# xswang/xflow

Measured on NVIDIA H100. Metric: training examples/sec, higher is better.
Workload: dtype f32

## Files before the change

xflow_b200/csrc/step_lazy.cu:

```cuda
#include <cuda_runtime.h>
#include <stdint.h>
#include <stdlib.h>

#include "kernels.h"
#include "table.cuh"

#define XF_NO_SLOT 0xFFFFFFFFu
#define XF_LAZY_CACHED 2

template <bool ADMIT, bool STAMP>
__device__ __forceinline__ bool xf_lazy_look(const XfTableView& t, uint64_t key, uint64_t& s, uint32_t& i, uint64_t& q0,
                                             uint64_t& q1, uint64_t& q2, uint64_t& q3, uint32_t& slot, bool& created,
                                             const XfAdmitView& adm, bool& rejected, const XfStampView& sv) {
  if (q0 == key) { slot = (uint32_t)s; return true; }
  if (q0 == XF_EMPTY_KEY) {
    if (ADMIT && !xf_admit(adm, key)) {
      rejected = adm.mode != XF_ADM_NEVER;
      return true;
    }
    const unsigned long long old =
        atomicCAS(reinterpret_cast<unsigned long long*>(xf_row(t, s)), (unsigned long long)XF_EMPTY_KEY, (unsigned long long)key);
    if (old == XF_EMPTY_KEY) {
      if (STAMP) sv.stamp[s] = sv.now;
      created = true;
      q0 = key; q1 = q2 = q3 = 0ull;
      slot = (uint32_t)s;
      return true;
    }
    if (old == key) {
      q0 = key;
      slot = (uint32_t)s;
      return true;
    }
  }
  if (++i == XF_MAX_PROBE) { *t.error = 1; return true; }
  s = xf_probe_slot(t, key, i);
  return false;
}

template <bool ADMIT, bool STAMP, bool WEIGHT>
__global__ void __launch_bounds__(256, 3)
xf_k_step_lr_lazy(XfTableView t, const uint32_t* __restrict__ row_ptr, const uint64_t* __restrict__ keys,
                  const uint8_t* __restrict__ labels, int B, int mode, uint32_t seq, uint64_t* rows_by_seq, int fix_shift,
                  float* __restrict__ loss_out, float* __restrict__ pctr_out, float* __restrict__ abs_loss_sum,
                  unsigned long long* __restrict__ unique_total, XfAdmitView adm, XfStampView sv, XfWeightView wv) {
  __shared__ float s_abs[8];
  __shared__ unsigned int s_open;
  if (WEIGHT) fix_shift = xf_fix_shift(*wv.W);
  __shared__ uint64_t s_q2[2 * XF_LAZY_CACHED][256], s_q3[2 * XF_LAZY_CACHED][256], s_q2n[2 * XF_LAZY_CACHED][256];
  if (threadIdx.x == 0) s_open = 0;
  if (blockIdx.x == 0 && threadIdx.x == 0 && mode == 0)
    rows_by_seq[seq] = (uint64_t)(uint32_t)B | ((uint64_t)fix_shift << 32);
  __syncthreads();
  float abs_acc = 0.f;
  unsigned int open_acc = 0;
  const int lane = threadIdx.x & 31;
  const int warps_per_block = blockDim.x >> 5;
  const int gwarp = blockIdx.x * warps_per_block + (threadIdx.x >> 5);
  const int nwarps = gridDim.x * warps_per_block;

  for (int row = gwarp; row < B; row += nwarps) {
    if (WEIGHT && __ldg(wv.e + row) == 0.f) {
      if (lane == 0 && loss_out) loss_out[row] = 0.f;
      continue;
    }
    const uint32_t beg = __ldg(row_ptr + row);
    const uint32_t end = __ldg(row_ptr + row + 1);
    const int chunks = (int)((end - beg + 63u) >> 6);
    float wsum = 0.f;
    uint32_t lead_s[2 * XF_LAZY_CACHED];
    uint32_t cnt_c[XF_LAZY_CACHED];
#pragma unroll
    for (int c = 0; c < XF_LAZY_CACHED; ++c) {
      lead_s[2 * c] = lead_s[2 * c + 1] = XF_NO_SLOT;
      cnt_c[c] = 0;
    }

    for (int ch = 0; ch < chunks; ++ch) {
      const uint32_t j0 = beg + (uint32_t)ch * 64u + (uint32_t)lane;
      const uint32_t j1 = j0 + 32u;
      const bool v0 = j0 < end, v1 = j1 < end;
      const uint64_t k0 = v0 ? __ldcs(keys + j0) : 0ull;
      const uint64_t k1 = v1 ? __ldcs(keys + j1) : 0ull;
      uint64_t p0 = xf_home_slot(t, k0), p1 = xf_home_slot(t, k1);
      uint64_t a0, a1, a2, a3, b0, b1, b2, b3;
      xf_ld32_pair(v0 ? xf_row(t, p0) : nullptr, a0, a1, a2, a3);
      xf_ld32_pair(v1 ? xf_row(t, p1) : nullptr, b0, b1, b2, b3);
      uint32_t s0 = XF_NO_SLOT, s1 = XF_NO_SLOT, i0 = 0, i1 = 0;
      bool u0 = v0, u1 = v1, r0 = false, r1 = false;
      for (;;) {
        bool c0 = false, c1 = false;
        if (u0) u0 = !xf_lazy_look<ADMIT, STAMP>(t, k0, p0, i0, a0, a1, a2, a3, s0, c0, adm, r0, sv);
        if (u1) u1 = !xf_lazy_look<ADMIT, STAMP>(t, k1, p1, i1, b0, b1, b2, b3, s1, c1, adm, r1, sv);
        const unsigned created = __popc(__ballot_sync(0xffffffffu, c0)) + __popc(__ballot_sync(0xffffffffu, c1));
        if (created && lane == 0) {
          atomicAdd(t.size, (unsigned long long)created);
          if (ADMIT) atomicAdd(adm.admitted, (unsigned long long)created);
        }
        if (!__any_sync(0xffffffffu, u0 || u1)) break;
        uint64_t x0, x1, x2, x3;
        xf_ld32_pair(u0 ? xf_row(t, p0) : nullptr, x0, x1, x2, x3);
        if (u0) { a0 = x0; a1 = x1; a2 = x2; a3 = x3; }
        xf_ld32_pair(u1 ? xf_row(t, p1) : nullptr, x0, x1, x2, x3);
        if (u1) { b0 = x0; b1 = x1; b2 = x2; b3 = x3; }
      }
      if (ADMIT) xf_admit_append(adm, r0, k0, r1, k1);
      uint64_t a2n = a2, b2n = b2;
      float w0 = 0.f, w1 = 0.f;
      if (s0 != XF_NO_SLOT) w0 = xf_lazy_fold(t, a1, a2, a3, mode == 1 ? 0xFFFFFFFFu : seq, a2n);
      if (s1 != XF_NO_SLOT) w1 = xf_lazy_fold(t, b1, b2, b3, mode == 1 ? 0xFFFFFFFFu : seq, b2n);
      wsum += w0;
      wsum += w1;
      if (mode == 1) continue;
      const unsigned grp0 = __match_any_sync(0xffffffffu, (s0 != XF_NO_SLOT) ? s0 : (0xFFFFFF00u | (uint32_t)lane));
      const unsigned grp1 = __match_any_sync(0xffffffffu, (s1 != XF_NO_SLOT) ? s1 : (0xFFFFFF00u | (uint32_t)lane));
      const bool L0 = s0 != XF_NO_SLOT && lane == __ffs(grp0) - 1, L1 = s1 != XF_NO_SLOT && lane == __ffs(grp1) - 1;
      if (ch >= XF_LAZY_CACHED) {
        if (L0 && xf_lazy_deposit(t, xf_row(t, s0), a2, a3, a2n, seq, 0ll)) {
          ++open_acc;
          if (STAMP) sv.stamp[s0] = sv.now;
        }
        if (L1 && xf_lazy_deposit(t, xf_row(t, s1), b2, b3, b2n, seq, 0ll)) {
          ++open_acc;
          if (STAMP) sv.stamp[s1] = sv.now;
        }
      }
#pragma unroll
      for (int c = 0; c < XF_LAZY_CACHED; ++c)
        if (ch == c) {
          lead_s[2 * c] = L0 ? s0 : XF_NO_SLOT;
          lead_s[2 * c + 1] = L1 ? s1 : XF_NO_SLOT;
          cnt_c[c] = (L0 ? (uint32_t)__popc(grp0) : 0u) | ((L1 ? (uint32_t)__popc(grp1) : 0u) << 8);
        }
      if (ch < XF_LAZY_CACHED) {
        if (L0) { s_q2[2 * ch][threadIdx.x] = a2; s_q3[2 * ch][threadIdx.x] = a3; s_q2n[2 * ch][threadIdx.x] = a2n; }
        if (L1) { s_q2[2 * ch + 1][threadIdx.x] = b2; s_q3[2 * ch + 1][threadIdx.x] = b3; s_q2n[2 * ch + 1][threadIdx.x] = b2n; }
      }
    }

    const float wx = xf_warp_sum(wsum);
    const float pctr = xf_sigmoid(wx);
    if (mode == 1) {
      if (lane == 0 && pctr_out) pctr_out[row] = pctr;
      continue;
    }
    float loss = __fsub_rn(pctr, (float)labels[row]);
    if (lane == 0 && loss_out) loss_out[row] = loss;
    if (WEIGHT) loss = __fmul_rn(__ldg(wv.e + row), loss);
    abs_acc += fabsf(loss);
    const long long lf = xf_fix_of(loss, fix_shift);
#pragma unroll
    for (int c = 0; c < XF_LAZY_CACHED; ++c) {
      const int x = threadIdx.x;
      if (lead_s[2 * c] != XF_NO_SLOT &&
          xf_lazy_deposit(t, xf_row(t, lead_s[2 * c]), s_q2[2 * c][x], s_q3[2 * c][x], s_q2n[2 * c][x], seq,
                          lf * (long long)(cnt_c[c] & 0xFFu))) {
        ++open_acc;
        if (STAMP) sv.stamp[lead_s[2 * c]] = sv.now;
      }
      if (lead_s[2 * c + 1] != XF_NO_SLOT &&
          xf_lazy_deposit(t, xf_row(t, lead_s[2 * c + 1]), s_q2[2 * c + 1][x], s_q3[2 * c + 1][x], s_q2n[2 * c + 1][x], seq,
                          lf * (long long)(cnt_c[c] >> 8))) {
        ++open_acc;
        if (STAMP) sv.stamp[lead_s[2 * c + 1]] = sv.now;
      }
    }
    for (int ch = XF_LAZY_CACHED; ch < chunks; ++ch) {
      const uint32_t j0 = beg + (uint32_t)ch * 64u + (uint32_t)lane;
      const uint32_t j1 = j0 + 32u;
      XfHead h;
      if (j0 < end) { const int64_t r = xf_probe<false>(t, __ldg(keys + j0), &h); if (r >= 0) xf_lazy_add(xf_row(t, (uint64_t)r), lf); }
      if (j1 < end) { const int64_t r = xf_probe<false>(t, __ldg(keys + j1), &h); if (r >= 0) xf_lazy_add(xf_row(t, (uint64_t)r), lf); }
    }
  }
  if (mode == 0) {
    if (lane == 0) s_abs[threadIdx.x >> 5] = abs_acc;
    if (open_acc) atomicAdd(&s_open, open_acc);
    __syncthreads();
    if (threadIdx.x == 0) {
      if (abs_loss_sum != nullptr) {
        float tot = 0.f;
        for (int w = 0; w < (int)(blockDim.x >> 5); ++w) tot += s_abs[w];
        atomicAdd(abs_loss_sum, tot);
      }
      if (unique_total != nullptr && s_open) atomicAdd(unique_total, (unsigned long long)s_open);
    }
  }
}

void xf_launch_step_lr_lazy(const XfTableView& t, const uint32_t* row_ptr, const uint64_t* keys,
                            const uint8_t* labels, int B, uint64_t nnz, int mode, uint32_t seq, uint64_t* rows_by_seq,
                            float* loss_out, float* pctr_out, float* abs_loss_sum, unsigned long long* unique_total,
                            const XfAdmitView* adm, const XfStampView& sv, const XfWeightView& wv, cudaStream_t st) {
  if (B <= 0) return;
  const int grid = xf_grid_for((uint64_t)B * 32, 256, 8);
  const int fs = xf_fix_shift(nnz);
  const XfAdmitView a = adm ? *adm : XfAdmitView{};
#define XF_LAZY_ARGS t, row_ptr, keys, labels, B, mode, seq, rows_by_seq, fs, loss_out, pctr_out, abs_loss_sum, unique_total, a, sv, wv
#define XF_LAZY_LAUNCH(A, S)                                                       \
  do {                                                                             \
    if (wv.e) xf_k_step_lr_lazy<A, S, true><<<grid, 256, 0, st>>>(XF_LAZY_ARGS);   \
    else xf_k_step_lr_lazy<A, S, false><<<grid, 256, 0, st>>>(XF_LAZY_ARGS);       \
  } while (0)
  const bool stamp = sv.stamp != nullptr;
  if (adm && stamp) XF_LAZY_LAUNCH(true, true);
  else if (adm) XF_LAZY_LAUNCH(true, false);
  else if (stamp) XF_LAZY_LAUNCH(false, true);
  else XF_LAZY_LAUNCH(false, false);
#undef XF_LAZY_LAUNCH
#undef XF_LAZY_ARGS
}
```

Baseline: 83.03 million.

## Prefetch second-chunk keys, split lazy deposits into issue/resolve, size grid by occupancy

Loads each row's label and its second chunk of keys before the first chunk's probe loop, so those loads overlap with hashing. Splits the cached-lead deposits into an issue phase for all groups followed by a resolve phase, so their memory operations can be in flight together. Relaxes launch bounds from 3 to 2 blocks per SM to allow more registers, and computes the grid from the measured occupancy instead of a fixed 8 blocks per SM. Holding the extra prefetched keys and in-flight values raises register pressure, and stale resolutions now set an error flag.

```diff
diff --git a/xflow_b200/csrc/step_lazy.cu b/xflow_b200/csrc/step_lazy.cu
--- a/xflow_b200/csrc/step_lazy.cu
+++ b/xflow_b200/csrc/step_lazy.cu
@@ -39,7 +39,7 @@
 }
 
 template <bool ADMIT, bool STAMP, bool WEIGHT>
-__global__ void __launch_bounds__(256, 3)
+__global__ void __launch_bounds__(256, 2)
 xf_k_step_lr_lazy(XfTableView t, const uint32_t* __restrict__ row_ptr, const uint64_t* __restrict__ keys,
                   const uint8_t* __restrict__ labels, int B, int mode, uint32_t seq, uint64_t* rows_by_seq, int fix_shift,
                   float* __restrict__ loss_out, float* __restrict__ pctr_out, float* __restrict__ abs_loss_sum,
@@ -67,6 +67,10 @@
     const uint32_t beg = __ldg(row_ptr + row);
     const uint32_t end = __ldg(row_ptr + row + 1);
     const int chunks = (int)((end - beg + 63u) >> 6);
+    const uint8_t label = mode == 0 ? labels[row] : 0;
+    uint64_t k1_0 = 0ull, k1_1 = 0ull;
+    if (beg + 64u + (uint32_t)lane < end) k1_0 = __ldcs(keys + beg + 64u + lane);
+    if (beg + 96u + (uint32_t)lane < end) k1_1 = __ldcs(keys + beg + 96u + lane);
     float wsum = 0.f;
     uint32_t lead_s[2 * XF_LAZY_CACHED];
     uint32_t cnt_c[XF_LAZY_CACHED];
@@ -80,8 +84,11 @@
       const uint32_t j0 = beg + (uint32_t)ch * 64u + (uint32_t)lane;
       const uint32_t j1 = j0 + 32u;
       const bool v0 = j0 < end, v1 = j1 < end;
-      const uint64_t k0 = v0 ? __ldcs(keys + j0) : 0ull;
-      const uint64_t k1 = v1 ? __ldcs(keys + j1) : 0ull;
+      uint64_t k0 = k1_0, k1 = k1_1;
+      if (ch != 1) {
+        k0 = v0 ? __ldcs(keys + j0) : 0ull;
+        k1 = v1 ? __ldcs(keys + j1) : 0ull;
+      }
       uint64_t p0 = xf_home_slot(t, k0), p1 = xf_home_slot(t, k1);
       uint64_t a0, a1, a2, a3, b0, b1, b2, b3;
       xf_ld32_pair(v0 ? xf_row(t, p0) : nullptr, a0, a1, a2, a3);
@@ -144,26 +151,30 @@
       if (lane == 0 && pctr_out) pctr_out[row] = pctr;
       continue;
     }
-    float loss = __fsub_rn(pctr, (float)labels[row]);
+    float loss = __fsub_rn(pctr, (float)label);
     if (lane == 0 && loss_out) loss_out[row] = loss;
     if (WEIGHT) loss = __fmul_rn(__ldg(wv.e + row), loss);
     abs_acc += fabsf(loss);
     const long long lf = xf_fix_of(loss, fix_shift);
-#pragma unroll
-    for (int c = 0; c < XF_LAZY_CACHED; ++c) {
+    uint64_t o2[2 * XF_LAZY_CACHED], o3[2 * XF_LAZY_CACHED];
+    bool issued[2 * XF_LAZY_CACHED];
+#pragma unroll
+    for (int g = 0; g < 2 * XF_LAZY_CACHED; ++g) {
       const int x = threadIdx.x;
-      if (lead_s[2 * c] != XF_NO_SLOT &&
-          xf_lazy_deposit(t, xf_row(t, lead_s[2 * c]), s_q2[2 * c][x], s_q3[2 * c][x], s_q2n[2 * c][x], seq,
-                          lf * (long long)(cnt_c[c] & 0xFFu))) {
+      issued[g] = lead_s[g] != XF_NO_SLOT &&
+                  xf_lazy_deposit_issue(xf_row(t, lead_s[g]), s_q2[g][x], s_q3[g][x], s_q2n[g][x], seq,
+                                        lf * (long long)((cnt_c[g >> 1] >> (8 * (g & 1))) & 0xFFu), o2[g], o3[g]);
+    }
+#pragma unroll
+    for (int g = 0; g < 2 * XF_LAZY_CACHED; ++g) {
+      const int x = threadIdx.x;
+      bool stale = false;
+      if (issued[g] && xf_lazy_deposit_resolve(xf_row(t, lead_s[g]), true, s_q2[g][x], s_q3[g][x], o2[g], o3[g], seq,
+                                               lf * (long long)((cnt_c[g >> 1] >> (8 * (g & 1))) & 0xFFu), &stale)) {
         ++open_acc;
-        if (STAMP) sv.stamp[lead_s[2 * c]] = sv.now;
-      }
-      if (lead_s[2 * c + 1] != XF_NO_SLOT &&
-          xf_lazy_deposit(t, xf_row(t, lead_s[2 * c + 1]), s_q2[2 * c + 1][x], s_q3[2 * c + 1][x], s_q2n[2 * c + 1][x], seq,
-                          lf * (long long)(cnt_c[c] >> 8))) {
-        ++open_acc;
-        if (STAMP) sv.stamp[lead_s[2 * c + 1]] = sv.now;
-      }
+        if (STAMP) sv.stamp[lead_s[g]] = sv.now;
+      }
+      if (stale) *t.error = 2;
     }
     for (int ch = XF_LAZY_CACHED; ch < chunks; ++ch) {
       const uint32_t j0 = beg + (uint32_t)ch * 64u + (uint32_t)lane;
@@ -188,25 +199,41 @@
   }
 }
 
+template <bool A, bool S, bool W>
+static int xf_lazy_ctas_per_sm() {
+  static const int n = [] {
+    int v = 0;
+    if (cudaOccupancyMaxActiveBlocksPerMultiprocessor(&v, xf_k_step_lr_lazy<A, S, W>, 256, 0) != cudaSuccess || v < 1) {
+      cudaGetLastError();
+      v = 1;
+    }
+    return v;
+  }();
+  return n;
+}
+
 void xf_launch_step_lr_lazy(const XfTableView& t, const uint32_t* row_ptr, const uint64_t* keys,
                             const uint8_t* labels, int B, uint64_t nnz, int mode, uint32_t seq, uint64_t* rows_by_seq,
                             float* loss_out, float* pctr_out, float* abs_loss_sum, unsigned long long* unique_total,
                             const XfAdmitView* adm, const XfStampView& sv, const XfWeightView& wv, cudaStream_t st) {
   if (B <= 0) return;
-  const int grid = xf_grid_for((uint64_t)B * 32, 256, 8);
   const int fs = xf_fix_shift(nnz);
   const XfAdmitView a = adm ? *adm : XfAdmitView{};
 #define XF_LAZY_ARGS t, row_ptr, keys, labels, B, mode, seq, rows_by_seq, fs, loss_out, pctr_out, abs_loss_sum, unique_total, a, sv, wv
-#define XF_LAZY_LAUNCH(A, S)                                                       \
-  do {                                                                             \
-    if (wv.e) xf_k_step_lr_lazy<A, S, true><<<grid, 256, 0, st>>>(XF_LAZY_ARGS);   \
-    else xf_k_step_lr_lazy<A, S, false><<<grid, 256, 0, st>>>(XF_LAZY_ARGS);       \
+#define XF_LAZY_LAUNCH(A, S, W)                                                                                      \
+  xf_k_step_lr_lazy<A, S, W><<<xf_grid_for((uint64_t)B * 32, 256, xf_lazy_ctas_per_sm<A, S, W>()), 256, 0, st>>>( \
+      XF_LAZY_ARGS)
+#define XF_LAZY_LAUNCH_W(A, S)            \
+  do {                                    \
+    if (wv.e) XF_LAZY_LAUNCH(A, S, true); \
+    else XF_LAZY_LAUNCH(A, S, false);     \
   } while (0)
   const bool stamp = sv.stamp != nullptr;
-  if (adm && stamp) XF_LAZY_LAUNCH(true, true);
-  else if (adm) XF_LAZY_LAUNCH(true, false);
-  else if (stamp) XF_LAZY_LAUNCH(false, true);
-  else XF_LAZY_LAUNCH(false, false);
+  if (adm && stamp) XF_LAZY_LAUNCH_W(true, true);
+  else if (adm) XF_LAZY_LAUNCH_W(true, false);
+  else if (stamp) XF_LAZY_LAUNCH_W(false, true);
+  else XF_LAZY_LAUNCH_W(false, false);
+#undef XF_LAZY_LAUNCH_W
 #undef XF_LAZY_LAUNCH
 #undef XF_LAZY_ARGS
 }
```

Result: faster. 87.18 million (median of 6 runs) (+5.0%).
